# AlexZou14/Wave-Mamba

Measured on AMD Instinct MI355X. Metric: UHD (3840x2160) images/sec fwd, higher is better.
Workload: dtype f32; 1 GPU; Wave-Mamba UHD-LL inference config (wf=32, n_l=[1,2,4], n_h=[1,1,2]), 1x3x2160x3840 reflect-padded to 2176x3840, seeded random init, one image per GPU per step, replicas (no collective); one forward at a time, its down-path high-frequency branches on side streams: True

## Files before the change

include/wavemamba_hip.h:

```cpp
#ifndef WAVEMAMBA_HIP_H
#define WAVEMAMBA_HIP_H

#include <stddef.h>
#include <stdint.h>

#ifdef __cplusplus
extern "C" {
#endif

#define WM_OK 0
#define WM_EINVAL (-1)
#define WM_ENULL (-2)
#define WM_EALIGN (-3)
#define WM_EWORKSPACE (-4)
#define WM_EUNSUPPORTED (-5)
#define WM_EHIP (-6)

#define WM_F32 0
#define WM_BF16 1

int wm_abi_version(void);
const char* wm_build_id(void);
const char* wm_strerror(int code);

// ... 78 lines not shown
size_t wm_conv2d_wfrag_bytes(int Cout, int Cin, int ks);
int wm_conv2d_prep(const float* weight, void* wfrag, int Cout, int Cin, int ks, void* stream);
int wm_conv2d_ln_fwd(const float* x, const float* ln_weight, const float* ln_bias, float ln_eps, const void* wfrag, const float* bias,
                     const float* residual, float* y, int B, int Cin, int Cout, int H, int W, void* stream);
int wm_dwconv_conv1x1_fwd(const float* x, int64_t x_batch_stride, const float* dw_weight, const float* dw_bias, int act,
                          const void* wfrag, const float* bias, const float* residual, float* y, int B, int C, int Cout, int H,
                          int W, void* stream);
int wm_conv2d_f16_steps(const float* x, const float* weight, const float* bias, float* y, float* amax, void* wfrag, int B, int Cin,
                        int Cout, int H, int W, int ks, int dgrad, void* stream);
int wm_conv2d_fwd(const float* xa, const float* xb, const int* xb_index, const void* wfrag, const float* bias,
                  const float* gate, const float* residual, float* y, int B, int Ca, int Cb, int Cb_src, int Cout,
                  int H, int W, int ks, void* stream);
int wm_conv2d_gated_fwd(const float* xa, const float* xb, const int* xb_index, const void* wfrag3, const void* wfrag1,
                        const float* bias1, float* y, int B, int Ca, int Cb, int Cb_src, int Cout, int H, int W,
                        void* stream);

size_t wm_ss2d_core_bwd_workspace_bytes(int B, int D, int H, int W, int N, int R);
int wm_ss2d_core_bwd(const float* x, const float* x_proj_weight, const float* dt_projs_weight,
                     const float* dt_projs_bias, const float* A_logs, const float* Ds, const float* dy_row_fwd,
                     const float* dy_row_rev, const float* dy_col_fwd, const float* dy_col_rev, float* dx,
                     float* dx_proj_weight, float* ddt_projs_weight, float* ddt_projs_bias, float* dA_logs, float* dDs,
                     void* workspace, size_t workspace_bytes, int B, int D, int H, int W, int N, int R, void* stream);

int wm_layernorm_tok_fwd(const float* x, const float* weight, const float* bias, float eps, float* y, int64_t T, int C,
                         void* stream);
int wm_layernorm_tok_bwd(const float* x, const float* weight, const float* gy, float eps, float* gx, float* dweight,
                         float* dbias, int64_t T, int C, void* stream);

int wm_image_pre_u8(const uint8_t* image, float* out, int h, int w, int Hp, int Wp, int swap_rb, void* stream);
int wm_image_post_u8(const float* in, uint8_t* image, int h, int w, int Hp, int Wp, int swap_rb, void* stream);
// ... 56 lines not shown
```

wave_mamba_amd/_lib.py:

```python
import ctypes
import os

HERE = os.path.dirname(os.path.abspath(__file__))
LIB_PATH = os.environ.get("WAVEMAMBA_HIP_LIB") or os.path.join(HERE, "libwavemamba_hip.so")

WM_F32, WM_BF16 = 0, 1
WM_OK, WM_EINVAL, WM_ENULL, WM_EALIGN, WM_EWORKSPACE, WM_EUNSUPPORTED, WM_EHIP = 0, -1, -2, -3, -4, -5, -6
WM_PROF_NKERNELS = 20
ABI_VERSION = 34

_c = ctypes
_p, _i, _i64, _sz = _c.c_void_p, _c.c_int, _c.c_int64, _c.c_size_t

SIGNATURES = {
    "wm_abi_version": (_i, []),
    "wm_build_id": (_c.c_char_p, []),
    "wm_strerror": (_c.c_char_p, [_i]),
    "wm_dwt2d_fwd": (_i, [_p] * 5 + [_i] * 5 + [_p]),
    "wm_dwt2d_bwd": (_i, [_p] * 5 + [_i] * 5 + [_p]),
    "wm_idwt2d_fwd": (_i, [_p] * 4 + [_i64] * 4 + [_p] + [_i] * 5 + [_p]),
    "wm_idwt2d_bwd": (_i, [_p] * 5 + [_i64] * 4 + [_i] * 5 + [_p]),
    "wm_selscan_fwd_workspace_bytes": (_sz, [_i] * 5),
    "wm_selscan_fwd": (_i, [_p] * 10 + [_p, _sz] + [_i] * 6 + [_p]),
    "wm_selscan_bwd_workspace_bytes": (_sz, [_i] * 5),
# ... 40 lines not shown
    "wm_gate_bwd": (_i, [_p] * 5 + [_i, _i] + [_i64] * 6 + [_p]),
    "wm_scale_add_fwd": (_i, [_p] * 4 + [_i, _i, _i64, _p]),
    "wm_scale_add_bwd": (_i, [_p] * 5 + [_i, _i, _i64, _p]),
    "wm_match_index": (_i, [_p, _p, _p, _p, _i, _i, _p]),
    "wm_attn_fold": (_i, [_p] * 6 + [_i, _i, _i, _p]),
    "wm_skff_workspace_bytes": (_sz, [_i, _i]),
    "wm_skff_fwd": (_i, [_p] * 7 + [_p, _sz] + [_i] * 5 + [_p]),
    "wm_conv2d_wfrag_bytes": (_sz, [_i, _i, _i]),
    "wm_conv2d_prep": (_i, [_p, _p, _i, _i, _i, _p]),
    "wm_conv2d_fwd": (_i, [_p] * 8 + [_i] * 8 + [_p]),
    "wm_conv2d_ln_fwd": (_i, [_p, _p, _p, _c.c_float, _p, _p, _p, _p] + [_i] * 5 + [_p]),
    "wm_dwconv_conv1x1_fwd": (_i, [_p, _i64, _p, _p, _i, _p, _p, _p, _p] + [_i] * 5 + [_p]),
    "wm_patchify_conv_fwd": (_i, [_p] * 4 + [_i] * 6 + [_p]),
    "wm_conv2d_f16_steps": (_i, [_p] * 6 + [_i] * 7 + [_p]),
    "wm_conv2d_gated_fwd": (_i, [_p] * 7 + [_i] * 7 + [_p]),
    "wm_conv2d_select": (_i, [_i]),
    "wm_prof_enable": (None, [ctypes.c_uint]),
    "wm_prof_collect": (_i, [_c.POINTER(_i), _c.POINTER(_c.c_double)]),
    "wm_event_synchronize_relaxed": (_i, [_p]),
    "wm_zero_arena_register": (_i, [_p, _c.c_size_t]),
    "wm_zero_arena_unregister": (_i, [_p]),
}

_lib = None


class WaveMambaHipError(RuntimeError):
    pass


# ... 37 lines not shown
```

wave_mamba_amd/archs/wavemamba_arch.py:

```python
import math

import os

import torch
import torch.nn as nn
import torch.nn.functional as F

try:
    from .. import ops as _hip_ops
    from ..registry import ARCH_REGISTRY
except ImportError:
    import wave_mamba_amd.ops as _hip_ops
    from basicsr.utils.registry import ARCH_REGISTRY


class _OpsBackend:
    impl = _hip_ops


def _op(name):
    return getattr(_OpsBackend.impl, name, None)


def _needs_grad(module, *tensors):
# ... 62 lines not shown

def _ln_conv(norm, conv, x):
    if norm is None:
        return _conv(conv, x)
    ops = _OpsBackend.impl
    if (_op("conv2d_ln") and ops.conv2d_ln_supported(x, conv.weight) and not _needs_grad(conv, x)
            and not _needs_grad(norm, x)):
        return ops.conv2d_ln(x, norm.weight, norm.bias, norm.eps, conv.weight, conv.bias)
    return _conv(conv, norm(x))


def _dw_pw_fused(x, dw_weight, pw_weight):
    ops = _OpsBackend.impl
    return bool(_op("dwconv_conv1x1") and ops.dwconv_conv1x1_supported(x, dw_weight, pw_weight)
                and _hip_ops._fuse_dw_pw_map(x.shape[0], x.shape[2], x.shape[3]))


def _cat_gathered(x, x2=None, x2_index=None):
    if x2 is None:
        return x
    if x2_index is not None:
        x2 = torch.gather(x2, 1, x2_index.long()[:, :, None, None].expand(-1, -1, x2.shape[2], x2.shape[3]))
    return torch.cat([x, x2], dim=1)


class DWT(nn.Module):

    def forward(self, x):
        return _OpsBackend.impl.dwt_init(x)

# ... 482 lines not shown

class DownFRG(nn.Module):

    early_qkv = True

    def __init__(self, dim, n_l_blocks=1, n_h_blocks=1, expand=2):
        super().__init__()
        self.dwt = DWT()
        self.l_conv = nn.Conv2d(dim * 2, dim, 3, 1, 1)
        self.l_blk = nn.Sequential(*[LFSSBlock(dim, expand=expand) for _ in range(n_l_blocks)])
        self.h_fusion = SKFF(dim, height=3, reduction=8)
        self.h_blk = nn.Sequential(*[HFEBlock(dim, match_factor=1, ffn_expansion_factor=1)
                                     for _ in range(n_h_blocks)])

    def forward(self, x, x_d, side=None, x_d_ready=None):
        ll, hl, lh, hh = self.dwt(x)
        if side is None:
            low = _run_lfss_stack(self.l_blk, _conv(self.l_conv, ll, x_d))
            high = self.h_fusion([hl, lh, hh])
            for blk in self.h_blk:
                high = blk(high, low)
            return low, high
        main = torch.cuda.current_stream(x.device)
        side.wait_stream(main)
        with torch.cuda.stream(side):
            high = self.h_fusion([hl, lh, hh])
            qkv0 = self.h_blk[0].qkv_of(high) if (len(self.h_blk) and self.early_qkv) else None
        if x_d_ready is not None:
            main.wait_event(x_d_ready)
            x_d.record_stream(main)
        low = _run_lfss_stack(self.l_blk, _conv(self.l_conv, ll, x_d))
        side.wait_stream(main)
        with torch.cuda.stream(side):
            for i, blk in enumerate(self.h_blk):
                high = blk(high, low, qkv=qkv0 if i == 0 else None)
        for t in (hl, lh, hh, low):
            t.record_stream(side)
        return low, high


class upFRG(nn.Module):

    def __init__(self, dim, n_l_blocks=1, n_h_blocks=1, expand=2):
        super().__init__()
        self.iwt = IWT()
        self.l_blk = nn.Sequential(*[LFSSBlock(dim, expand=expand) for _ in range(n_l_blocks)])
        self.h_out_conv = nn.Conv2d(dim, dim * 3, 3, 1, 1)
        self.h_blk = nn.Sequential(*[HFEBlock(dim, match_factor=1, ffn_expansion_factor=1)
                                     for _ in range(n_h_blocks)])

    def forward(self, x_l, x_h, join=None):
        low = _run_lfss_stack(self.l_blk, x_l)
        qkv0 = None
        if join is not None:
            x_h, qkv0 = join(x_h)
        for i, blk in enumerate(self.h_blk):
            x_h = blk(x_h, low, qkv=qkv0 if i == 0 else None)
        return self.iwt(low, _conv(self.h_out_conv, x_h))


_SIDE_STREAMS = {}


def _side_streams(x, n):
    if not x.is_cuda:
        return (None,) * n
    dev = x.device.index if x.device.index is not None else torch.cuda.current_device()
    capturing = torch.cuda.is_current_stream_capturing()
    key = (dev, "capture" if capturing else torch.cuda.current_stream(x.device).cuda_stream)
    sts = _SIDE_STREAMS.get(key)
    if sts is None or len(sts) < n:
        if capturing:
            raise RuntimeError("WaveMamba: run one eager forward on this device before capturing it into a graph "
# ... 29 lines not shown
        pss = (self.ps_down1, self.ps_down2, self.ps_down3)
        ops = _OpsBackend.impl
        fused_ps = _op("patchify_conv") and all(ops.patchify_conv_supported(img, ps[1].weight, ps[0].downscale_factor)
                                                for ps in pss)
        if sides[0] is None or fused_ps:
            d, d_ready = [_ps_conv(ps, img) for ps in pss], (None, None, None)
        else:
            main = torch.cuda.current_stream(x.device)
            d, d_ready = [], []
            for ps, side in zip(pss, sides):
                side.wait_stream(main)
                with torch.cuda.stream(side):
                    d.append(_ps_conv(ps, img))
                    d_ready.append(side.record_event())
            img.record_stream(sides[0]); img.record_stream(sides[1]); img.record_stream(sides[2])
        low, high1 = self.down_group1(_conv(self.conv_01, img), d[0], sides[0], d_ready[0])
        low, high2 = self.down_group2(low, d[1], sides[1], d_ready[1])
        low, high3 = self.down_group3(low, d[2], sides[2], d_ready[2])

        def joiner(side, up_group, high):
            if side is None:
                return None
            with torch.cuda.stream(side):
                qkv = up_group.h_blk[0].qkv_of(high) if len(up_group.h_blk) else None

            def join(high):
                main = torch.cuda.current_stream(x.device)
                main.wait_stream(side)
                for t in (high, *(qkv if isinstance(qkv, tuple) else (qkv,))):
                    if t is not None:
                        t.record_stream(main)
                return high, qkv
            return join
        low = self.up_group3(low, high3, joiner(sides[2], self.up_group3, high3))
        low = self.up_group2(low, high2, joiner(sides[1], self.up_group2, high2))
        low = self.up_group1(low, high1, joiner(sides[0], self.up_group1, high1))
        return _conv(self.last, low, residual=img)


@ARCH_REGISTRY.register()
class WaveMamba(nn.Module):

    scale_factor = 1

    def __init__(self, *, in_chn, wf, n_l_blocks=[1, 1, 2], n_h_blocks=[1, 1, 1], ffn_scale=2.0,
                 **ignore_kwargs):
        super().__init__()
        self.restoration_network = UNet(in_chn=in_chn, wf=wf, n_l_blocks=n_l_blocks,
                                        n_h_blocks=n_h_blocks, ffn_scale=ffn_scale)

# ... 44 lines not shown
```

wave_mamba_amd/csrc/conv.hip:

```cpp
#include "host_common.h"
#include "conv2d.hip.h"
#include "conv2d_ws.hip.h"
#include "patchify.hip.h"
#include "dw_pw.hip.h"

using namespace wm;

template <int KS, int RW, int MT, bool G1X1 = false, bool F16 = false, bool LNIN = false>
static int conv2d_launch(const wm::Conv2dArgs& a, int B, hipStream_t st) {
    constexpr int PAD = KS / 2;
    constexpr int smem = ((4 * RW + 2 * PAD) * (wm::kCvTW + 2 * PAD) * 4 + (KS * KS + (G1X1 ? 1 : 0)) * MT * 2 * 64) * 16;
    static bool configured[64] = {};
    if (smem > 65536) {
        const int rc = wm::lds_optin((const void*)wm::conv2d_mfma_kernel<KS, RW, MT, G1X1, F16, LNIN>, smem, configured);
        if (rc) return rc;
    }
    const int ntiles = ((a.W + wm::kCvTW - 1) / wm::kCvTW) * ((a.H + 4 * RW - 1) / (4 * RW));
    const dim3 grid((unsigned)(((ntiles + 7) / 8) * 8), (unsigned)B);
    hipLaunchKernelGGL((wm::conv2d_mfma_kernel<KS, RW, MT, G1X1, F16, LNIN>), grid, dim3(256), smem, st, a);
    return launch_status();
}

#ifndef WM_CONV_WS_RW2
#define WM_CONV_WS_RW2 4
// ... 9 lines not shown
#endif
static std::atomic<int> g_conv_select{0};
static int conv_select_mode() { return g_conv_select.load(std::memory_order_relaxed); }
static bool conv_ws_enabled(const wm::Conv2dArgs& a, int B, int th) {
    const int mode = conv_select_mode();
    if (mode == 1) return false;
    const long long cmax = std::max(std::max(a.Ca, a.xb ? a.Cbsrc : 0), a.Cout);
    if (cmax * a.H * a.W * 4 >= (1ll << 32) || (a.xb_idx && a.Cb > 128)) return false;
    if (a.gate && a.res) return false;
    if (mode == 2) return true;
    if ((a.gate || a.res) && a.mtot > 1) return false;
    const long long ntiles = (long long)B * ((a.W + wm::kWsTW - 1) / wm::kWsTW) * ((a.H + th - 1) / th);
    return ntiles >= 768;
}

template <int RW, int MT, bool G1X1 = false, bool EPI = false, int NPW = 4, bool F16 = false>
static int conv2d_ws_launch(const wm::Conv2dArgs& a, int B, hipStream_t st) {
    using Cfg = wm::ConvWsCfg<RW, MT, G1X1, NPW>;
    static bool configured[64] = {};
    static int ncu[64] = {};
    static std::mutex mu;
    int dev = 0;
    if (hipGetDevice(&dev) != hipSuccess || dev < 0 || dev >= 64) return WM_EHIP;
    {
        std::lock_guard<std::mutex> lk(mu);
        if (!configured[dev]) {
            if (hipFuncSetAttribute((const void*)wm::conv3x3_ws_kernel<RW, MT, G1X1, EPI, NPW, F16>, hipFuncAttributeMaxDynamicSharedMemorySize,
                                    Cfg::LDS_BYTES) != hipSuccess) return WM_EHIP;
            if (hipDeviceGetAttribute(&ncu[dev], hipDeviceAttributeMultiprocessorCount, dev) != hipSuccess) return WM_EHIP;
            configured[dev] = true;
        }
    }
    const long long ntiles = (long long)B * ((a.W + wm::kWsTW - 1) / wm::kWsTW) * ((a.H + Cfg::TH - 1) / Cfg::TH);
    if (ntiles >= (1ll << 31)) return WM_EUNSUPPORTED;
    const int cus = std::max(8, ncu[dev] & ~7);
    const int G = (int)std::min<long long>(cus, ((ntiles + 7) / 8) * 8);
    hipLaunchKernelGGL((wm::conv3x3_ws_kernel<RW, MT, G1X1, EPI, NPW, F16>), dim3((unsigned)G), dim3(256 + 64 * NPW), Cfg::LDS_BYTES, st, a, B);
    return launch_status();
}

extern "C" {

int wm_patchify_conv_fwd(const float* img, const float* weight, const float* bias, float* y, int B, int Cin, int Cout, int H, int W,
                         int r, void* stream) {
    if (B < 0 || Cin <= 0 || Cout <= 0 || H < 0 || W < 0) return WM_EINVAL;
    if (r != 2 && r != 4 && r != 8) return WM_EUNSUPPORTED;
    if (H % r || W % r) return WM_EINVAL;
    if (Cout != 16 && Cout != 32 && Cout != 48 && Cout != 64) return WM_EUNSUPPORTED;
    const size_t lds = (size_t)Cin * r * r * Cout * sizeof(float);
    if (lds > 64 * 1024) return WM_EUNSUPPORTED;
    if (B == 0 || H == 0 || W == 0) return WM_OK;
    if (!img || !weight || !y) return WM_ENULL;
// ... 182 lines not shown
    hipStream_t st = (hipStream_t)stream;
    if (zero_out(amax, 2 * sizeof(float), st) != hipSuccess) return WM_EHIP;
    const long long nx = (long long)B * Cin * H * W, nw = (long long)Cout * Cin * ks * ks;
    long long blocks = (nx / 4 + 256 * 8 - 1) / (256 * 8);
    blocks = blocks < 1 ? 1 : (blocks > 512 ? 512 : blocks);
    const int nch = (Cin + 15) / 16, mtot = (Cout + 31) / 32;
    const long long items = (long long)nch * ks * ks * mtot * 128;
    const int nprep = (int)(items <= 512 ? 1 : (items >= 32 * 512 ? 32 : (items + 511) / 512));
    hipLaunchKernelGGL(cv_amax_prep_kernel, dim3((unsigned)blocks + nprep), dim3(256), 0, st, x, nx, weight, nw, (unsigned*)amax,
                       (uint4*)wfrag, Cout, Cin, ks * ks, nch, mtot, dgrad ? 1 : 0, nprep);
    int rc = launch_status();
    if (rc) return rc;
    return conv2d_fwd_f16(x, wfrag, amax, bias, y, B, Cin, Cout, H, W, ks, stream);
}

int wm_conv2d_gated_fwd(const float* xa, const float* xb, const int* xb_index, const void* wfrag3, const void* wfrag1,
                        const float* bias1, float* y, int B, int Ca, int Cb, int Cb_src, int Cout, int H, int W,
                        void* stream) {
    if (B < 0 || Ca <= 0 || Cb < 0 || Cout <= 0 || H < 0 || W < 0 || Cb_src < 0) return WM_EINVAL;
    if (B == 0 || H == 0 || W == 0) return WM_OK;
    if (!xa || !wfrag3 || !wfrag1 || !y || (Cb > 0 && !xb)) return WM_ENULL;
    if (Cb > 0 && Ca % 8 != 0) return WM_EUNSUPPORTED;
    if (Cb > 0 && !xb_index && Cb_src != Cb) return WM_EINVAL;
    if (B > 65535 || (long long)H * W >= (1ll << 31)) return WM_EUNSUPPORTED;
    if (!aligned16(wfrag3) || !aligned16(wfrag1)) return WM_EALIGN;
    hipStream_t st = (hipStream_t)stream;
    Conv2dArgs a;
    a.xa = xa; a.xb = Cb > 0 ? xb : nullptr; a.xb_idx = Cb > 0 ? xb_index : nullptr; a.wfrag = (const uint4*)wfrag3;
    a.bias = nullptr; a.gate = nullptr; a.res = nullptr; a.y = y; a.wfrag1 = (const uint4*)wfrag1; a.bias1 = bias1;
    a.Ca = Ca; a.Cb = Cb; a.Cbsrc = Cb_src; a.Cout = Cout; a.H = H; a.W = W;
// ... 30 lines not shown
```

wave_mamba_amd/csrc/conv2d.hip.h:

```cpp
#pragma once
#include <hip/hip_runtime.h>
#include <stdint.h>

namespace wm {

using bf16x8_t = __attribute__((ext_vector_type(8))) __bf16;
using f16x8_t = __attribute__((ext_vector_type(8))) _Float16;
using f32x16_t = __attribute__((ext_vector_type(16))) float;

constexpr int kCvTW = 32;

struct Conv2dArgs {
    const float* xa;
    const float* xb;
    const int* xb_idx;
    const uint4* wfrag;
    const float* bias;
    const float* gate;
    const float* res;
    const uint4* wfrag1;
    const float* bias1;
    float* y;
    int Ca, Cb, Cbsrc, Cout, H, W;
    int nch;
    int mtot;
    int mbase;
    const float* amax;
    const float* ln_w;
    const float* ln_b;
    float ln_eps;
};

union Frag16 {
    bf16x8_t v;
    f16x8_t h;
    uint4 u;
};
// ... 403 lines not shown
```

wave_mamba_amd/csrc/conv2d_ws.hip.h:

```cpp
#pragma once
#include <type_traits>
#include "conv2d.hip.h"

namespace wm {

constexpr int kWsTW = 64;

template <int RW, int MT, bool G1X1, int NPW = 4>
struct ConvWsCfg {
    static constexpr int NPT = 64 * NPW;
    static constexpr int PW = kWsTW + 2;
    static constexpr int TH = 2 * RW;
    static constexpr int NPIX = (TH + 2) * PW;
    static constexpr int PIT = (NPIX + NPT - 1) / NPT;
    static constexpr int W_ITEMS = 9 * MT * 2 * 64;
    static constexpr int W1_ITEMS = G1X1 ? MT * 2 * 64 : 0;
    static constexpr int BUF_ITEMS = 4 * NPIX + W_ITEMS + W1_ITEMS;
    static constexpr int LDS_BYTES = 2 * BUF_ITEMS * 16 + 2 * MT * 32 * 4;
};

struct ConvWsTiles {
    int tiles_x, ntiles_img, first, stride, count;
    __device__ ConvWsTiles(int B, int H, int W, int TH, int g, int G) {
        tiles_x = (W + kWsTW - 1) / kWsTW;
// ... 22 lines not shown
#define CV_STAMP(role, it, k) do { if (WM_CV_STAMP && blockIdx.x == 0 && lane == 0 && (wave & 3) == 0 && (it) < 128) \
        g_cv_stamps[((role) * 128 + (it)) * 8 + (k)] = __builtin_readcyclecounter(); } while (0)
#else
#define CV_STAMP(role, it, k) do { } while (0)
#endif

using u32x4_t = __attribute__((ext_vector_type(4))) unsigned;
template <int OFF>
__device__ __forceinline__ void ws_lds_store16(unsigned addr, const uint4& v) {
    u32x4_t d = {v.x, v.y, v.z, v.w};
    asm volatile("ds_write_b128 %0, %1 offset:%2" : : "v"(addr), "v"(d), "n"(OFF) : "memory");
}

__device__ __forceinline__ void ws_barrier_lds() { asm volatile("s_waitcnt lgkmcnt(0)\n\ts_barrier" ::: "memory"); }

template <int RW, int MT, bool G1X1, bool EPI, int NPW = 4, bool F16 = false>
__global__ __launch_bounds__(256 + 64 * NPW, (4 + NPW) / 4) void conv3x3_ws_kernel(const Conv2dArgs a, const int B) {
    extern __shared__ __attribute__((aligned(16))) unsigned char cv_smem[];
    static_assert(!(F16 && G1X1), "the fp16 form (conv2d.hip.h) serves the plain convolutions of the training step");
    const float sx = F16 ? cv_pow2_scale(a.amax[0]) : 1.0f;
    const float osc = F16 ? 1.0f / (sx * cv_pow2_scale(a.amax[1])) : 1.0f;
    using Cfg = ConvWsCfg<RW, MT, G1X1, NPW>;
    constexpr int PW = Cfg::PW, TH = Cfg::TH, NPIX = Cfg::NPIX, PIT = Cfg::PIT, NPT = Cfg::NPT;
    constexpr int W_ITEMS = Cfg::W_ITEMS, W1_ITEMS = Cfg::W1_ITEMS, BUF = Cfg::BUF_ITEMS;
    uint4* const smem = reinterpret_cast<uint4*>(cv_smem);

    const int tid = threadIdx.x, lane = tid & 63;
    const int wave = __builtin_amdgcn_readfirstlane(tid >> 6);
    const ConvWsTiles tl(B, a.H, a.W, TH, (int)blockIdx.x, (int)gridDim.x);
    if (tl.count == 0) return;
    const int nch = a.nch;
    const int n_it = tl.count * nch;
    const int H = a.H, W = a.W;
    const long long HW = (long long)H * W;

    if (tid < 2 * MT * 32) {
        const int which = tid / (MT * 32), ch = a.mbase * 32 + tid % (MT * 32);
        const float* src = which ? a.bias1 : a.bias;
        reinterpret_cast<float*>(smem + 2 * BUF)[tid] = (src && ch < a.Cout) ? src[ch] : 0.0f;
    }
    if (wave >= 4) {
        const int ptid = tid - 256, pw = wave - 4;
        const unsigned lds_base = (unsigned)(size_t)(__attribute__((address_space(3))) unsigned char*)cv_smem;
        static_assert(2 * NPIX * 16 < 65536, "the lo plane sits within the ds_write offset field");
        float pin[2][2][PIT][8];
        unsigned okm[2][PIT];
        int ccs[2] = {0, 0};
        unsigned poff[PIT];
        unsigned okF[PIT];
        int jf = -1, ccf = nch - 1;
        const float* xaF = a.xa;
        const float* xbF = a.xa;
        int idxv0 = 0, idxv1 = 0, bF = -1;

        auto fetch_w = [&](int buf, int cc) {
            uint4* s_w = smem + buf * BUF + 4 * NPIX;
            const uint4* wsrc = a.wfrag + ((long long)cc * 9 * a.mtot) * 128;
            constexpr int W_IT = (W_ITEMS + NPT - 1) / NPT;
#pragma unroll
            for (int it = 0; it < W_IT; ++it) {
// ... 9 lines not shown
                uint4* s_w1 = s_w + W_ITEMS;
                const uint4* w1src = a.wfrag1 + ((long long)cc * a.mtot) * 128;
                const int item0 = pw * 64;
                if (item0 < W1_ITEMS) {
                    const uint4* g = w1src + (a.mbase + (item0 >> 7)) * 128 + (item0 & 64) + lane;
                    __builtin_amdgcn_global_load_lds((const __attribute__((address_space(1))) void*)g,
                                                     (__attribute__((address_space(3))) void*)(s_w1 + item0), 16, 0, 0);
                }
            }
        };
        auto advance = [&]() {
            if (++ccf == nch) {
                ccf = 0; ++jf;
                int b, h0, w0;
                tl.locate(jf, TH, b, h0, w0);
#pragma unroll
                for (int it = 0; it < PIT; ++it) {
                    const int p = ptid + it * NPT;
                    const int pr = p / PW, pc = p - pr * PW;
                    const int h = h0 - 1 + pr, w = w0 - 1 + pc;
                    const bool ok = p < NPIX && h >= 0 && h < H && w >= 0 && w < W;
                    okF[it] = ok ? 0xffffffffu : 0u;
                    poff[it] = ok ? (unsigned)(h * W + w) * 4u : 0u;
                    asm volatile("" : "+v"(okF[it]), "+v"(poff[it]));
                }
                if (b != bF) {
                    bF = b;
                    xaF = a.xa + (long long)b * a.Ca * HW;
                    xbF = a.xb ? a.xb + (long long)b * a.Cbsrc * HW : a.xa;
                    if (a.xb_idx) {
                        const int* idx = a.xb_idx + (long long)b * a.Cb;
                        idxv0 = lane < a.Cb ? idx[lane] : 0;
                        idxv1 = lane + 64 < a.Cb ? idx[lane + 64] : 0;
                        asm volatile("" : "+v"(idxv0), "+v"(idxv1));
                    }
                }
            }
        };
        auto fetch_half = [&](auto SETC, auto HALFC) {
            constexpr int S = decltype(SETC)::value, half = decltype(HALFC)::value;
            if (half == 0) {
                ccs[S] = ccf;
#pragma unroll
                for (int it = 0; it < PIT; ++it) okm[S][it] = okF[it];
            }
            const int c0 = ccf * 16 + half * 8;
            const bool from_a = c0 < a.Ca;
            const int cl = from_a ? c0 : c0 - a.Ca;
            const int cn = (from_a ? a.Ca : a.Cb) - cl;
            const char* src = reinterpret_cast<const char*>(from_a ? xaF : xbF);
            const bool gather = !from_a && a.xb_idx;
#pragma unroll
            for (int j = 0; j < 8; ++j) {
                const bool cok = j < cn;
                const int cg = cl + j;
                const int ch = !cok ? 0 : !gather ? cg
                             : cg < 64 ? __builtin_amdgcn_readlane(idxv0, cg) : __builtin_amdgcn_readlane(idxv1, cg - 64);
                const unsigned choff = (unsigned)ch * (unsigned)HW * 4u;
#pragma unroll
                for (int it = 0; it < PIT; ++it)
                    pin[S][half][it][j] = *reinterpret_cast<const float*>(src + (size_t)(choff + poff[it]));
            }
        };
        auto stage_half = [&](auto SETC, auto HALFC, int buf) {
            constexpr int S = decltype(SETC)::value, half = decltype(HALFC)::value;
            const unsigned s_in = lds_base + (unsigned)(buf * BUF + half * NPIX + ptid) * 16u;
            const int c0 = ccs[S] * 16 + half * 8;
            const int cn = c0 < a.Ca ? a.Ca - c0 : a.Ca + a.Cb - c0;
#pragma unroll
            for (int it = 0; it < PIT; ++it) {
                const int p = ptid + it * NPT;
                if (NPIX % NPT == 0 || p < NPIX) {
                    Frag16 hi, lo;
#pragma unroll
                    for (int j = 0; j < 8; ++j) {
                        const float v = j < cn ? __builtin_bit_cast(float, __builtin_bit_cast(unsigned, pin[S][half][it][j]) & okm[S][it]) : 0.0f;
                        cv_split<F16>(F16 ? v * sx : v, hi, lo, j);
                    }
                    ws_lds_store16<0>(s_in + it * (NPT * 16u), hi.u);
                    ws_lds_store16<2 * NPIX * 16>(s_in + it * (NPT * 16u), lo.u);
                }
            }
        };
        using C0 = std::integral_constant<int, 0>;
        using C1 = std::integral_constant<int, 1>;
        auto step = [&](auto SF, auto SS, bool do_fetch, bool do_stage, int buf, int i) {
            CV_STAMP(1, i, 0);
            if (do_stage) fetch_w(buf, ccs[decltype(SS)::value]);
            if (do_fetch) { advance(); fetch_half(SF, C0{}); }
            CV_STAMP(1, i, 1);
            if (do_stage) stage_half(SS, C0{}, buf);
            if (do_fetch) fetch_half(SF, C1{});
            CV_STAMP(1, i, 2);
            if (do_stage) stage_half(SS, C1{}, buf);
            __builtin_amdgcn_s_waitcnt(0x0070);
// ... 164 lines not shown
                const int h = h0 + rg * RW + r;
                if (h >= H || w >= W) continue;
                const long long o = (((long long)b * a.Cout + chb) * H + h) * W + w;
#pragma unroll
                for (int i = 0; i < 16; ++i) {
                    const int dc = (i & 3) + 8 * (i >> 2);
                    float v = (F16 ? acc[m][r][i] * osc : acc[m][r][i]) + bv[i];
                    if constexpr (G1X1) v = v / (1.0f + __expf(-(acc1[m][r][i] + b1v[i])));
                    if constexpr (EPI) v = is_gate ? v / (1.0f + __expf(-ev[r][i])) : v + ev[r][i];
                    if (full || chb + dc < a.Cout) a.y[o + dc * HW] = v;
                }
            }
        }
    };

    ws_barrier_lds();
    int cc = 0, j = 0;
    for (int i = 0; i < n_it; ++i) {
        CV_STAMP(0, i, 0);
        mma(i & 1);
        CV_STAMP(0, i, 1);
        ws_barrier_lds();
        CV_STAMP(0, i, 2);
        if (++cc == nch) {
            epilogue(j, M0{});
            if (MT > 1) epilogue(j, M1{});
            zero_acc(M0{});
            if (MT > 1) zero_acc(M1{});
            cc = 0; ++j;
        }
        CV_STAMP(0, i, 3);
    }
}

}
```

wave_mamba_amd/ops.py:

```python
import os
import weakref

import torch
import torch.nn.functional as F

from . import _lib
from ._lib import WM_BF16, WM_F32, check


def _stream():
    return torch.cuda.current_stream().cuda_stream


def _require_cuda(name, *tensors):
    for t in tensors:
        if t is not None and not t.is_cuda:
            raise RuntimeError(
                f"{name}: expected a CUDA (ROCm) tensor, got device '{t.device}'. The Wave-Mamba hot "
                "path is HIP-only (dwt_init / iwt_init / selective_scan_fn alone have a CPU twin, for inputs that are ALL "
                "on the CPU); nothing falls back to the CPU.")


def _dtype_code(t, name):
    if t.dtype == torch.float32:
# ... 1038 lines not shown
        raise ValueError(f"dwconv_conv1x1: act must be 'none' or 'gelu', got {act!r}")
    B, C, H, W = x.shape
    if residual is not None and (tuple(residual.shape) != (B, 32, H, W) or residual.dtype != torch.float32):
        raise RuntimeError(f"dwconv_conv1x1: residual must be float32 {(B, 32, H, W)}, got {tuple(residual.shape)}")
    if tuple(x.stride()[1:]) != (H * W, W, 1) or (B > 1 and x.stride(0) < C * H * W):
        x = x.contiguous()
    frag = _conv2d_wfrag(weight, cache=not dynamic_weight)
    y = torch.empty((B, 32, H, W), dtype=torch.float32, device=x.device)
    _launch(x.device, "wm_dwconv_conv1x1_fwd", x, x.stride(0) if B > 1 else C * H * W, _w(dw_weight),
            None if dw_bias is None else _w(dw_bias), {"none": 0, "gelu": 2}[act], frag,
            None if bias is None else bias.detach().contiguous(), None if residual is None else residual.contiguous(), y,
            B, C, 32, H, W)
    return y


def patchify_conv_supported(img, weight, r):
    return (img.is_cuda and img.dtype == torch.float32 and img.dim() == 4 and weight.dim() == 4 and r in (2, 4, 8)
            and tuple(weight.shape[2:]) == (1, 1) and weight.shape[1] == img.shape[1] * r * r and weight.shape[0] in (16, 32, 48, 64)
            and img.shape[2] % r == 0 and img.shape[3] % r == 0 and weight.shape[0] * weight.shape[1] <= 16384)


def patchify_conv(img, weight, bias, r):
    _require_cuda("patchify_conv", img, weight)
    if not patchify_conv_supported(img, weight, r):
        raise ValueError("patchify_conv: unsupported shapes (see patchify_conv_supported)")
    img = img.contiguous()
    B, Cin, H, W = img.shape
    Cout = weight.shape[0]
    y = torch.empty((B, Cout, H // r, W // r), dtype=torch.float32, device=img.device)
    _launch(img.device, "wm_patchify_conv_fwd", img, _w(weight), None if bias is None else _w(bias), y, B, Cin, Cout, H, W, r)
# ... 317 lines not shown
```

Before: 34.55 images/s.

## Fuse first conv with Haar DWT and inverse DWT with last conv

Adds a conv3x3 variant whose epilogue applies the forward Haar transform across lane pairs via DPP and writes the four half-resolution bands directly. It also adds a variant whose producer stage loads low/high bands and synthesises full-resolution pixels into LDS before the last convolution. The model uses these for conv_01+DWT and IWT+last conv at UHD resolution. This removes the full-resolution 32-channel intermediate write and read at both ends of the network, at the cost of more complex producer and epilogue code.

```diff
diff --git a/include/wavemamba_hip.h b/include/wavemamba_hip.h
--- a/include/wavemamba_hip.h
+++ b/include/wavemamba_hip.h
@@ -116,6 +116,10 @@
 int wm_conv2d_gated_fwd(const float* xa, const float* xb, const int* xb_index, const void* wfrag3, const void* wfrag1,
                         const float* bias1, float* y, int B, int Ca, int Cb, int Cb_src, int Cout, int H, int W,
                         void* stream);
+int wm_conv2d_dwt_fwd(const void* img, const void* wfrag, const float* bias, void* ll, void* hl, void* lh, void* hh, int B, int Cin,
+                      int Cout, int H, int W, int dtype, void* stream);
+int wm_idwt_conv2d_fwd(const void* low, const void* high, const void* wfrag, const float* bias, const float* residual, float* y, int B,
+                       int Cin, int Cout, int H, int W, int dtype, void* stream);
 
 size_t wm_ss2d_core_bwd_workspace_bytes(int B, int D, int H, int W, int N, int R);
 int wm_ss2d_core_bwd(const float* x, const float* x_proj_weight, const float* dt_projs_weight,
diff --git a/wave_mamba_amd/_lib.py b/wave_mamba_amd/_lib.py
--- a/wave_mamba_amd/_lib.py
+++ b/wave_mamba_amd/_lib.py
@@ -78,6 +78,8 @@
     "wm_patchify_conv_fwd": (_i, [_p] * 4 + [_i] * 6 + [_p]),
     "wm_conv2d_f16_steps": (_i, [_p] * 6 + [_i] * 7 + [_p]),
     "wm_conv2d_gated_fwd": (_i, [_p] * 7 + [_i] * 7 + [_p]),
+    "wm_conv2d_dwt_fwd": (_i, [_p] * 7 + [_i] * 6 + [_p]),
+    "wm_idwt_conv2d_fwd": (_i, [_p] * 6 + [_i] * 6 + [_p]),
     "wm_conv2d_select": (_i, [_i]),
     "wm_prof_enable": (None, [ctypes.c_uint]),
     "wm_prof_collect": (_i, [_c.POINTER(_i), _c.POINTER(_c.c_double)]),
diff --git a/wave_mamba_amd/archs/wavemamba_arch.py b/wave_mamba_amd/archs/wavemamba_arch.py
--- a/wave_mamba_amd/archs/wavemamba_arch.py
+++ b/wave_mamba_amd/archs/wavemamba_arch.py
@@ -100,6 +100,24 @@
     ops = _OpsBackend.impl
     return bool(_op("dwconv_conv1x1") and ops.dwconv_conv1x1_supported(x, dw_weight, pw_weight)
                 and _hip_ops._fuse_dw_pw_map(x.shape[0], x.shape[2], x.shape[3]))
+
+
+def _conv_dwt_fused(conv, img):
+    ops = _OpsBackend.impl
+    return bool(_op("conv2d_dwt") and ops.conv2d_dwt_supported(img, conv.weight) and not _needs_grad(conv, img)
+                and _hip_ops._fuse_conv_dwt_map(img.shape[0], img.shape[2], img.shape[3]))
+
+
+def _conv_dwt(conv, img):
+    if _conv_dwt_fused(conv, img):
+        return _OpsBackend.impl.conv2d_dwt(img, conv.weight, conv.bias)
+    return _conv(conv, img)
+
+
+def _iwt_conv_fused(net, conv, low, out_like):
+    ops = _OpsBackend.impl
+    return bool(_op("iwt_conv2d") and ops.iwt_conv2d_supported(low, conv.weight) and not _needs_grad(net, low, out_like)
+                and _hip_ops._fuse_iwt_conv_map(out_like.shape[0], out_like.shape[2], out_like.shape[3]))
 
 
 def _cat_gathered(x, x2=None, x2_index=None):
@@ -612,14 +630,14 @@
                                      for _ in range(n_h_blocks)])
 
     def forward(self, x, x_d, side=None, x_d_ready=None):
-        ll, hl, lh, hh = self.dwt(x)
+        ll, hl, lh, hh = x if isinstance(x, tuple) else self.dwt(x)
         if side is None:
             low = _run_lfss_stack(self.l_blk, _conv(self.l_conv, ll, x_d))
             high = self.h_fusion([hl, lh, hh])
             for blk in self.h_blk:
                 high = blk(high, low)
             return low, high
-        main = torch.cuda.current_stream(x.device)
+        main = torch.cuda.current_stream(ll.device)
         side.wait_stream(main)
         with torch.cuda.stream(side):
             high = self.h_fusion([hl, lh, hh])
@@ -647,14 +665,15 @@
         self.h_blk = nn.Sequential(*[HFEBlock(dim, match_factor=1, ffn_expansion_factor=1)
                                      for _ in range(n_h_blocks)])
 
-    def forward(self, x_l, x_h, join=None):
+    def forward(self, x_l, x_h, join=None, synthesise=True):
         low = _run_lfss_stack(self.l_blk, x_l)
         qkv0 = None
         if join is not None:
             x_h, qkv0 = join(x_h)
         for i, blk in enumerate(self.h_blk):
             x_h = blk(x_h, low, qkv=qkv0 if i == 0 else None)
-        return self.iwt(low, _conv(self.h_out_conv, x_h))
+        high = _conv(self.h_out_conv, x_h)
+        return self.iwt(low, high) if synthesise else (low, high)
 
 
 _SIDE_STREAMS = {}
@@ -714,7 +733,7 @@
                     d.append(_ps_conv(ps, img))
                     d_ready.append(side.record_event())
             img.record_stream(sides[0]); img.record_stream(sides[1]); img.record_stream(sides[2])
-        low, high1 = self.down_group1(_conv(self.conv_01, img), d[0], sides[0], d_ready[0])
+        low, high1 = self.down_group1(_conv_dwt(self.conv_01, img), d[0], sides[0], d_ready[0])
         low, high2 = self.down_group2(low, d[1], sides[1], d_ready[1])
         low, high3 = self.down_group3(low, d[2], sides[2], d_ready[2])
 
@@ -734,6 +753,9 @@
             return join
         low = self.up_group3(low, high3, joiner(sides[2], self.up_group3, high3))
         low = self.up_group2(low, high2, joiner(sides[1], self.up_group2, high2))
+        if _iwt_conv_fused(self, self.last, low, img):
+            low, high = self.up_group1(low, high1, joiner(sides[0], self.up_group1, high1), synthesise=False)
+            return ops.iwt_conv2d(low, high, self.last.weight, self.last.bias, img)
         low = self.up_group1(low, high1, joiner(sides[0], self.up_group1, high1))
         return _conv(self.last, low, residual=img)
 
diff --git a/wave_mamba_amd/csrc/conv.hip b/wave_mamba_amd/csrc/conv.hip
--- a/wave_mamba_amd/csrc/conv.hip
+++ b/wave_mamba_amd/csrc/conv.hip
@@ -47,7 +47,7 @@
     return ntiles >= 768;
 }
 
-template <int RW, int MT, bool G1X1 = false, bool EPI = false, int NPW = 4, bool F16 = false>
+template <int RW, int MT, bool G1X1 = false, bool EPI = false, int NPW = 4, bool F16 = false, bool DWTE = false, bool IWTI = false>
 static int conv2d_ws_launch(const wm::Conv2dArgs& a, int B, hipStream_t st) {
     using Cfg = wm::ConvWsCfg<RW, MT, G1X1, NPW>;
     static bool configured[64] = {};
@@ -58,7 +58,7 @@
     {
         std::lock_guard<std::mutex> lk(mu);
         if (!configured[dev]) {
-            if (hipFuncSetAttribute((const void*)wm::conv3x3_ws_kernel<RW, MT, G1X1, EPI, NPW, F16>, hipFuncAttributeMaxDynamicSharedMemorySize,
+            if (hipFuncSetAttribute((const void*)wm::conv3x3_ws_kernel<RW, MT, G1X1, EPI, NPW, F16, DWTE, IWTI>, hipFuncAttributeMaxDynamicSharedMemorySize,
                                     Cfg::LDS_BYTES) != hipSuccess) return WM_EHIP;
             if (hipDeviceGetAttribute(&ncu[dev], hipDeviceAttributeMultiprocessorCount, dev) != hipSuccess) return WM_EHIP;
             configured[dev] = true;
@@ -68,7 +68,7 @@
     if (ntiles >= (1ll << 31)) return WM_EUNSUPPORTED;
     const int cus = std::max(8, ncu[dev] & ~7);
     const int G = (int)std::min<long long>(cus, ((ntiles + 7) / 8) * 8);
-    hipLaunchKernelGGL((wm::conv3x3_ws_kernel<RW, MT, G1X1, EPI, NPW, F16>), dim3((unsigned)G), dim3(256 + 64 * NPW), Cfg::LDS_BYTES, st, a, B);
+    hipLaunchKernelGGL((wm::conv3x3_ws_kernel<RW, MT, G1X1, EPI, NPW, F16, DWTE, IWTI>), dim3((unsigned)G), dim3(256 + 64 * NPW), Cfg::LDS_BYTES, st, a, B);
     return launch_status();
 }
 
@@ -281,6 +281,53 @@
     return conv2d_fwd_f16(x, wfrag, amax, bias, y, B, Cin, Cout, H, W, ks, stream);
 }
 
+int wm_conv2d_dwt_fwd(const void* img, const void* wfrag, const float* bias, void* ll, void* hl, void* lh, void* hh, int B, int Cin,
+                      int Cout, int H, int W, int dtype, void* stream) {
+    if (B < 0 || Cin <= 0 || Cout <= 0 || H < 0 || W < 0) return WM_EINVAL;
+    if (H % 2 || W % 2) return WM_EINVAL;
+    if (dtype != WM_F32 || Cout != 32) return WM_EUNSUPPORTED;
+    if (B == 0 || H == 0 || W == 0) return WM_OK;
+    if (!img || !wfrag || !ll || !hl || !lh || !hh) return WM_ENULL;
+    if (B > 65535 || (long long)H * W >= (1ll << 31)) return WM_EUNSUPPORTED;
+    if (!aligned16(wfrag)) return WM_EALIGN;
+    hipStream_t st = (hipStream_t)stream;
+    Conv2dArgs a;
+    a.xa = (const float*)img; a.xb = nullptr; a.xb_idx = nullptr; a.wfrag = (const uint4*)wfrag;
+    a.bias = bias; a.gate = nullptr; a.res = nullptr; a.wfrag1 = nullptr; a.bias1 = nullptr;
+    a.y = (float*)ll; a.yband[0] = (float*)hl; a.yband[1] = (float*)lh; a.yband[2] = (float*)hh;
+    a.Ca = Cin; a.Cb = 0; a.Cbsrc = 0; a.Cout = Cout; a.H = H; a.W = W;
+    a.nch = (Cin + 15) / 16; a.mtot = 1; a.mbase = 0; a.amax = nullptr; a.ln_w = nullptr; a.ln_b = nullptr; a.ln_eps = 0.0f;
+    if (conv_select_mode() == 1 || (long long)std::max(Cin, Cout) * H * W * 4 >= (1ll << 32)) return WM_EUNSUPPORTED;
+    ProfScope ps(13, st);
+    return conv2d_ws_launch<WM_CONV_WS_RW1, 1, false, false, WM_CONV_WS_NPW1, false, true>(a, B, st);
+}
+
+int wm_idwt_conv2d_fwd(const void* low, const void* high, const void* wfrag, const float* bias, const float* residual, float* y, int B,
+                       int Cin, int Cout, int H, int W, int dtype, void* stream) {
+    if (B < 0 || Cin <= 0 || Cout <= 0 || H < 0 || W < 0) return WM_EINVAL;
+    if (H % 2 || W % 2) return WM_EINVAL;
+    if (dtype != WM_F32 || Cin != 32) return WM_EUNSUPPORTED;
+    if (B == 0 || H == 0 || W == 0) return WM_OK;
+    if (!low || !high || !wfrag || !y) return WM_ENULL;
+    if (B > 65535 || (long long)H * W >= (1ll << 31)) return WM_EUNSUPPORTED;
+    if (!aligned16(wfrag)) return WM_EALIGN;
+    hipStream_t st = (hipStream_t)stream;
+    Conv2dArgs a;
+    a.xa = (const float*)low; a.xb = (const float*)high; a.xb_idx = nullptr; a.wfrag = (const uint4*)wfrag;
+    a.bias = bias; a.gate = nullptr; a.res = residual; a.y = y; a.wfrag1 = nullptr; a.bias1 = nullptr;
+    a.Ca = Cin; a.Cb = 0; a.Cbsrc = 3 * Cin; a.Cout = Cout; a.H = H; a.W = W;
+    a.nch = Cin / 16; a.mtot = (Cout + 31) / 32; a.amax = nullptr; a.ln_w = nullptr; a.ln_b = nullptr; a.ln_eps = 0.0f;
+    if (conv_select_mode() == 1 || (long long)std::max(Cin, Cout) * H * W * 4 >= (1ll << 32)) return WM_EUNSUPPORTED;
+    ProfScope ps(13, st);
+    for (int mb = 0; mb < a.mtot; ++mb) {
+        a.mbase = mb;
+        const int rc = residual ? conv2d_ws_launch<WM_CONV_WS_RW1, 1, false, true, 4, false, false, true>(a, B, st)
+                                : conv2d_ws_launch<WM_CONV_WS_RW1, 1, false, false, WM_CONV_WS_NPW1, false, false, true>(a, B, st);
+        if (rc) return rc;
+    }
+    return WM_OK;
+}
+
 int wm_conv2d_gated_fwd(const float* xa, const float* xb, const int* xb_index, const void* wfrag3, const void* wfrag1,
                         const float* bias1, float* y, int B, int Ca, int Cb, int Cb_src, int Cout, int H, int W,
                         void* stream) {
diff --git a/wave_mamba_amd/csrc/conv2d.hip.h b/wave_mamba_amd/csrc/conv2d.hip.h
--- a/wave_mamba_amd/csrc/conv2d.hip.h
+++ b/wave_mamba_amd/csrc/conv2d.hip.h
@@ -21,6 +21,7 @@
     const uint4* wfrag1;
     const float* bias1;
     float* y;
+    float* yband[3] = {nullptr, nullptr, nullptr};
     int Ca, Cb, Cbsrc, Cout, H, W;
     int nch;
     int mtot;
diff --git a/wave_mamba_amd/csrc/conv2d_ws.hip.h b/wave_mamba_amd/csrc/conv2d_ws.hip.h
--- a/wave_mamba_amd/csrc/conv2d_ws.hip.h
+++ b/wave_mamba_amd/csrc/conv2d_ws.hip.h
@@ -1,6 +1,7 @@
 #pragma once
 #include <type_traits>
 #include "conv2d.hip.h"
+#include "haar.hip.h"
 
 namespace wm {
 
@@ -60,10 +61,16 @@
 
 __device__ __forceinline__ void ws_barrier_lds() { asm volatile("s_waitcnt lgkmcnt(0)\n\ts_barrier" ::: "memory"); }
 
-template <int RW, int MT, bool G1X1, bool EPI, int NPW = 4, bool F16 = false>
+__device__ __forceinline__ float ws_from_pair_lane(float v) {
+    return __builtin_bit_cast(float, __builtin_amdgcn_update_dpp(0, __builtin_bit_cast(int, v), 0xB1, 0xf, 0xf, false));
+}
+
+template <int RW, int MT, bool G1X1, bool EPI, int NPW = 4, bool F16 = false, bool DWTE = false, bool IWTI = false>
 __global__ __launch_bounds__(256 + 64 * NPW, (4 + NPW) / 4) void conv3x3_ws_kernel(const Conv2dArgs a, const int B) {
     extern __shared__ __attribute__((aligned(16))) unsigned char cv_smem[];
     static_assert(!(F16 && G1X1), "the fp16 form (conv2d.hip.h) serves the plain convolutions of the training step");
+    static_assert(!DWTE || (MT == 1 && !G1X1 && !EPI && !F16 && RW % 2 == 0), "the analysis epilogue: one plain 32-channel row tile, whole quads per wave");
+    static_assert(!IWTI || (!G1X1 && !F16), "the synthesis staging: the plain bf16 form");
     const float sx = F16 ? cv_pow2_scale(a.amax[0]) : 1.0f;
     const float osc = F16 ? 1.0f / (sx * cv_pow2_scale(a.amax[1])) : 1.0f;
     using Cfg = ConvWsCfg<RW, MT, G1X1, NPW>;
@@ -89,7 +96,13 @@
         const int ptid = tid - 256, pw = wave - 4;
         const unsigned lds_base = (unsigned)(size_t)(__attribute__((address_space(3))) unsigned char*)cv_smem;
         static_assert(2 * NPIX * 16 < 65536, "the lo plane sits within the ds_write offset field");
-        float pin[2][2][PIT][8];
+        constexpr int QR = (TH + 4) / 2, QC = (kWsTW + 4) / 2;
+        static_assert(!IWTI || QR * QC <= NPT, "one quad per producer thread");
+        constexpr int PSL = IWTI ? 4 : PIT;
+        const int qr = IWTI ? ptid / QC : 0, qc = IWTI ? ptid - qr * QC : 0;
+        const int h2 = IWTI ? a.H >> 1 : 0, w2 = IWTI ? a.W >> 1 : 0;
+        const unsigned HW2b = IWTI ? (unsigned)(h2 * w2) * 4u : 0u;
+        float pin[2][2][PSL][8];
         unsigned okm[2][PIT];
         int ccs[2] = {0, 0};
         unsigned poff[PIT];
@@ -129,20 +142,28 @@
                 ccf = 0; ++jf;
                 int b, h0, w0;
                 tl.locate(jf, TH, b, h0, w0);
-#pragma unroll
-                for (int it = 0; it < PIT; ++it) {
-                    const int p = ptid + it * NPT;
-                    const int pr = p / PW, pc = p - pr * PW;
-                    const int h = h0 - 1 + pr, w = w0 - 1 + pc;
-                    const bool ok = p < NPIX && h >= 0 && h < H && w >= 0 && w < W;
-                    okF[it] = ok ? 0xffffffffu : 0u;
-                    poff[it] = ok ? (unsigned)(h * W + w) * 4u : 0u;
-                    asm volatile("" : "+v"(okF[it]), "+v"(poff[it]));
+                if constexpr (IWTI) {
+                    const int qh = (h0 >> 1) - 1 + qr, qw = (w0 >> 1) - 1 + qc;
+                    const bool ok = qr < QR && qh >= 0 && qh < h2 && qw >= 0 && qw < w2;
+                    okF[0] = ok ? 0xffffffffu : 0u;
+                    poff[0] = ok ? (unsigned)(qh * w2 + qw) * 4u : 0u;
+                    asm volatile("" : "+v"(okF[0]), "+v"(poff[0]));
+                } else {
+#pragma unroll
+                    for (int it = 0; it < PIT; ++it) {
+                        const int p = ptid + it * NPT;
+                        const int pr = p / PW, pc = p - pr * PW;
+                        const int h = h0 - 1 + pr, w = w0 - 1 + pc;
+                        const bool ok = p < NPIX && h >= 0 && h < H && w >= 0 && w < W;
+                        okF[it] = ok ? 0xffffffffu : 0u;
+                        poff[it] = ok ? (unsigned)(h * W + w) * 4u : 0u;
+                        asm volatile("" : "+v"(okF[it]), "+v"(poff[it]));
+                    }
                 }
                 if (b != bF) {
                     bF = b;
-                    xaF = a.xa + (long long)b * a.Ca * HW;
-                    xbF = a.xb ? a.xb + (long long)b * a.Cbsrc * HW : a.xa;
+                    xaF = a.xa + (long long)b * a.Ca * (IWTI ? (long long)h2 * w2 : HW);
+                    xbF = a.xb ? a.xb + (long long)b * a.Cbsrc * (IWTI ? (long long)h2 * w2 : HW) : a.xa;
                     if (a.xb_idx) {
                         const int* idx = a.xb_idx + (long long)b * a.Cb;
                         idxv0 = lane < a.Cb ? idx[lane] : 0;
@@ -157,43 +178,82 @@
             if (half == 0) {
                 ccs[S] = ccf;
 #pragma unroll
-                for (int it = 0; it < PIT; ++it) okm[S][it] = okF[it];
+                for (int it = 0; it < (IWTI ? 1 : PIT); ++it) okm[S][it] = okF[it];
             }
             const int c0 = ccf * 16 + half * 8;
-            const bool from_a = c0 < a.Ca;
-            const int cl = from_a ? c0 : c0 - a.Ca;
-            const int cn = (from_a ? a.Ca : a.Cb) - cl;
-            const char* src = reinterpret_cast<const char*>(from_a ? xaF : xbF);
-            const bool gather = !from_a && a.xb_idx;
-#pragma unroll
-            for (int j = 0; j < 8; ++j) {
-                const bool cok = j < cn;
-                const int cg = cl + j;
-                const int ch = !cok ? 0 : !gather ? cg
-                             : cg < 64 ? __builtin_amdgcn_readlane(idxv0, cg) : __builtin_amdgcn_readlane(idxv1, cg - 64);
-                const unsigned choff = (unsigned)ch * (unsigned)HW * 4u;
-#pragma unroll
-                for (int it = 0; it < PIT; ++it)
-                    pin[S][half][it][j] = *reinterpret_cast<const float*>(src + (size_t)(choff + poff[it]));
+            if constexpr (IWTI) {
+                const char* lowp = reinterpret_cast<const char*>(xaF);
+                const char* highp = reinterpret_cast<const char*>(xbF);
+#pragma unroll
+                for (int j = 0; j < 8; ++j) {
+                    pin[S][half][0][j] = *reinterpret_cast<const float*>(lowp + (size_t)((unsigned)(c0 + j) * HW2b + poff[0]));
+#pragma unroll
+                    for (int k = 0; k < 3; ++k)
+                        pin[S][half][1 + k][j] =
+                            *reinterpret_cast<const float*>(highp + (size_t)((unsigned)(k * a.Ca + c0 + j) * HW2b + poff[0]));
+                }
+            } else {
+                const bool from_a = c0 < a.Ca;
+                const int cl = from_a ? c0 : c0 - a.Ca;
+                const int cn = (from_a ? a.Ca : a.Cb) - cl;
+                const char* src = reinterpret_cast<const char*>(from_a ? xaF : xbF);
+                const bool gather = !from_a && a.xb_idx;
+#pragma unroll
+                for (int j = 0; j < 8; ++j) {
+                    const bool cok = j < cn;
+                    const int cg = cl + j;
+                    const int ch = !cok ? 0 : !gather ? cg
+                                 : cg < 64 ? __builtin_amdgcn_readlane(idxv0, cg) : __builtin_amdgcn_readlane(idxv1, cg - 64);
+                    const unsigned choff = (unsigned)ch * (unsigned)HW * 4u;
+#pragma unroll
+                    for (int it = 0; it < PIT; ++it)
+                        pin[S][half][it][j] = *reinterpret_cast<const float*>(src + (size_t)(choff + poff[it]));
+                }
             }
         };
         auto stage_half = [&](auto SETC, auto HALFC, int buf) {
             constexpr int S = decltype(SETC)::value, half = decltype(HALFC)::value;
-            const unsigned s_in = lds_base + (unsigned)(buf * BUF + half * NPIX + ptid) * 16u;
-            const int c0 = ccs[S] * 16 + half * 8;
-            const int cn = c0 < a.Ca ? a.Ca - c0 : a.Ca + a.Cb - c0;
-#pragma unroll
-            for (int it = 0; it < PIT; ++it) {
-                const int p = ptid + it * NPT;
-                if (NPIX % NPT == 0 || p < NPIX) {
-                    Frag16 hi, lo;
-#pragma unroll
-                    for (int j = 0; j < 8; ++j) {
-                        const float v = j < cn ? __builtin_bit_cast(float, __builtin_bit_cast(unsigned, pin[S][half][it][j]) & okm[S][it]) : 0.0f;
-                        cv_split<F16>(F16 ? v * sx : v, hi, lo, j);
-                    }
-                    ws_lds_store16<0>(s_in + it * (NPT * 16u), hi.u);
-                    ws_lds_store16<2 * NPIX * 16>(s_in + it * (NPT * 16u), lo.u);
+            if constexpr (IWTI) {
+                const unsigned s_q = lds_base + (unsigned)(buf * BUF + half * NPIX + (2 * qr - 1) * PW + 2 * qc - 1) * 16u;
+                float px4[4][8];
+#pragma unroll
+                for (int j = 0; j < 8; ++j) {
+                    float sb[4];
+#pragma unroll
+                    for (int k = 0; k < 4; ++k)
+                        sb[k] = __builtin_bit_cast(float, __builtin_bit_cast(unsigned, pin[S][half][k][j]) & okm[S][0]);
+                    haar_inv<false>(sb[0], sb[1], sb[2], sb[3], px4[0][j], px4[1][j], px4[2][j], px4[3][j]);
+                }
+#pragma unroll
+                for (int q = 0; q < 4; ++q) {
+                    const int dr = q & 1, dc = q >> 1;
+                    const bool in = qr < QR && (dr ? qr < QR - 1 : qr > 0) && (dc ? qc < QC - 1 : qc > 0);
+                    if (in) {
+                        Frag16 hi, lo;
+#pragma unroll
+                        for (int j = 0; j < 8; ++j) cv_split<false>(px4[q][j], hi, lo, j);
+                        const unsigned ad = s_q + (unsigned)(dr * PW + dc) * 16u;
+                        ws_lds_store16<0>(ad, hi.u);
+                        ws_lds_store16<2 * NPIX * 16>(ad, lo.u);
+                    }
+                }
+            } else {
+                const unsigned s_in = lds_base + (unsigned)(buf * BUF + half * NPIX + ptid) * 16u;
+                const int c0 = ccs[S] * 16 + half * 8;
+                const int cn = c0 < a.Ca ? a.Ca - c0 : a.Ca + a.Cb - c0;
+#pragma unroll
+                for (int it = 0; it < PIT; ++it) {
+                    const int p = ptid + it * NPT;
+                    if (NPIX % NPT == 0 || p < NPIX) {
+                        Frag16 hi, lo;
+#pragma unroll
+                        for (int j = 0; j < 8; ++j) {
+                            const float v = j < cn ? __builtin_bit_cast(float, __builtin_bit_cast(unsigned, pin[S][half][it][j]) & okm[S][it]) : 0.0f;
+                            cv_split<F16>(F16 ? v * sx : v, hi, lo, j);
+                        }
+                        ws_lds_store16<0>(s_in + it * (NPT * 16u), hi.u);
+                        ws_lds_store16<2 * NPIX * 16>(s_in + it * (NPT * 16u), lo.u);
+                    }
                 }
             }
         };
@@ -388,6 +448,45 @@
         }
     };
 
+    auto epilogue_dwt = [&](int j) {
+        int b, h0, w0;
+        const bool fast = tile_fast(j, b, h0, w0);
+        const int w = w0 + cw * 32 + px, hq = (h0 + rg * RW) >> 1;
+        const bool odd = px & 1;
+        const int h2 = H >> 1, w2 = W >> 1;
+        const unsigned HW2b = (unsigned)(h2 * w2) * 4u;
+        const size_t bo = (size_t)b * a.Cout * HW2b;
+        char* const y0 = reinterpret_cast<char*>(odd ? a.yband[1] : a.y) + bo;
+        char* const y1 = reinterpret_cast<char*>(odd ? a.yband[2] : a.yband[0]) + bo;
+        const int chb = a.mbase * 32 + 4 * khalf;
+        const unsigned o0 = (unsigned)((chb * h2 + hq) * w2 + (w >> 1)) * 4u;
+        float bv[16];
+#pragma unroll
+        for (int i = 0; i < 16; ++i) bv[i] = s_bias[4 * khalf + (i & 3) + 8 * (i >> 2)];
+        auto quads = [&](auto FASTC) {
+            constexpr bool FAST = decltype(FASTC)::value;
+#pragma unroll
+            for (int rp = 0; rp < RW / 2; ++rp) {
+                const bool in = FAST || (h0 + rg * RW + 2 * rp < H && w < W);
+#pragma unroll
+                for (int i = 0; i < 16; ++i) {
+                    const int dc = (i & 3) + 8 * (i >> 2);
+                    const float v0 = acc[0][2 * rp][i] + bv[i], v1 = acc[0][2 * rp + 1][i] + bv[i];
+                    const float n0 = ws_from_pair_lane(v0), n1 = ws_from_pair_lane(v1);
+                    float ll, hl, lh, hh;
+                    haar_fwd<false>(odd ? n0 : v0, odd ? n1 : v1, odd ? v0 : n0, odd ? v1 : n1, ll, hl, lh, hh);
+                    const unsigned o = o0 + (unsigned)(rp * w2) * 4u + (unsigned)dc * HW2b;
+                    if (FAST || (in && (full || chb + dc < a.Cout))) {
+                        *reinterpret_cast<float*>(y0 + (size_t)o) = odd ? lh : ll;
+                        *reinterpret_cast<float*>(y1 + (size_t)o) = odd ? hh : hl;
+                    }
+                }
+            }
+        };
+        if (fast) quads(std::true_type{});
+        else quads(std::false_type{});
+    };
+
     ws_barrier_lds();
     int cc = 0, j = 0;
     for (int i = 0; i < n_it; ++i) {
@@ -397,8 +496,11 @@
         ws_barrier_lds();
         CV_STAMP(0, i, 2);
         if (++cc == nch) {
-            epilogue(j, M0{});
-            if (MT > 1) epilogue(j, M1{});
+            if constexpr (DWTE) epilogue_dwt(j);
+            else {
+                epilogue(j, M0{});
+                if (MT > 1) epilogue(j, M1{});
+            }
             zero_acc(M0{});
             if (MT > 1) zero_acc(M1{});
             cc = 0; ++j;
diff --git a/wave_mamba_amd/ops.py b/wave_mamba_amd/ops.py
--- a/wave_mamba_amd/ops.py
+++ b/wave_mamba_amd/ops.py
@@ -1076,6 +1076,71 @@
     return y
 
 
+_FUSE_CONV_DWT = True
+_FUSE_CONV_DWT_MIN_POSITIONS = 1088 * 1920
+
+
+def _fuse_conv_dwt_map(B, H, W):
+    return _FUSE_CONV_DWT and B == 1 and H * W >= _FUSE_CONV_DWT_MIN_POSITIONS
+
+
+def conv2d_dwt_supported(x, weight):
+    return (x.is_cuda and x.dim() == 4 and weight.dim() == 4 and tuple(weight.shape) == (32, x.shape[1], 3, 3)
+            and x.dtype == torch.float32 and weight.dtype == torch.float32 and x.shape[2] % 2 == 0 and x.shape[3] % 2 == 0
+            and x.shape[0] <= 65535 and max(32, x.shape[1]) * x.shape[2] * x.shape[3] * 4 < 2 ** 32)
+
+
+def conv2d_dwt(x, weight, bias=None):
+    _require_cuda("conv2d_dwt", x, weight, bias)
+    if not conv2d_dwt_supported(x, weight):
+        raise NotImplementedError("conv2d_dwt: fp32, a (32, Cin, 3, 3) weight, even H and W, the wave-specialised 3x3 kernel's limits")
+    B, Cin, H, W = x.shape
+    x = x.contiguous()
+    frag = _conv2d_wfrag(weight)
+    outs = [torch.empty((B, 32, H // 2, W // 2), dtype=torch.float32, device=x.device) for _ in range(4)]
+    rc = _launch(x.device, "wm_conv2d_dwt_fwd", x, frag, None if bias is None else bias.detach().contiguous(), *outs, B, Cin, 32, H, W,
+                 WM_F32, status=True)
+    if rc == _lib.WM_EUNSUPPORTED:
+        return dwt_init(conv2d(x, weight, bias))
+    check(rc, "wm_conv2d_dwt_fwd")
+    return tuple(outs)
+
+
+_FUSE_IWT_CONV = True
+_FUSE_IWT_CONV_MIN_POSITIONS = 1088 * 1920
+
+
+def _fuse_iwt_conv_map(B, H, W):
+    return _FUSE_IWT_CONV and B == 1 and H * W >= _FUSE_IWT_CONV_MIN_POSITIONS
+
+
+def iwt_conv2d_supported(low, weight):
+    return (low.is_cuda and low.dim() == 4 and low.shape[1] == 32 and weight.dim() == 4 and tuple(weight.shape[1:]) == (32, 3, 3)
+            and low.dtype == torch.float32 and weight.dtype == torch.float32 and low.shape[0] <= 65535
+            and max(32, weight.shape[0]) * low.shape[2] * low.shape[3] * 16 < 2 ** 32)
+
+
+def iwt_conv2d(low, high, weight, bias=None, residual=None):
+    _require_cuda("iwt_conv2d", low, high, weight, bias, residual)
+    if not iwt_conv2d_supported(low, weight):
+        raise NotImplementedError("iwt_conv2d: fp32, 32-channel bands, a (Cout, 32, 3, 3) weight, the wave-specialised 3x3 kernel's limits")
+    B, C, h, w = low.shape
+    cout = weight.shape[0]
+    if tuple(high.shape) != (B, 3 * C, h, w) or high.dtype != torch.float32:
+        raise RuntimeError(f"iwt_conv2d: high must be float32 {(B, 3 * C, h, w)}, got {tuple(high.shape)}")
+    if residual is not None and (tuple(residual.shape) != (B, cout, 2 * h, 2 * w) or residual.dtype != torch.float32):
+        raise RuntimeError(f"iwt_conv2d: residual must be float32 {(B, cout, 2 * h, 2 * w)}, got {tuple(residual.shape)}")
+    frag = _conv2d_wfrag(weight)
+    y = torch.empty((B, cout, 2 * h, 2 * w), dtype=torch.float32, device=low.device)
+    rc = _launch(low.device, "wm_idwt_conv2d_fwd", low.contiguous(), high.contiguous(), frag,
+                 None if bias is None else bias.detach().contiguous(), None if residual is None else residual.contiguous(), y,
+                 B, C, cout, 2 * h, 2 * w, WM_F32, status=True)
+    if rc == _lib.WM_EUNSUPPORTED:
+        return conv2d(iwt_init_pair(low, high), weight, bias, residual=residual)
+    check(rc, "wm_idwt_conv2d_fwd")
+    return y
+
+
 def patchify_conv_supported(img, weight, r):
     return (img.is_cuda and img.dtype == torch.float32 and img.dim() == 4 and weight.dim() == 4 and r in (2, 4, 8)
             and tuple(weight.shape[2:]) == (1, 1) and weight.shape[1] == img.shape[1] * r * r and weight.shape[0] in (16, 32, 48, 64)
```

Measured after the change: 35.14 images/s (median of 6 runs). 1.7% higher.
